# acg-team/ProGraphMSA

Hardware: AMD Instinct MI355X
Metric: DP cell-updates/sec (GCUPS) + wall-clock on 256 seqs × 1000 aa, WAG (higher is better)
Workload: dtype f32

## Files before the change

include/pgm_hip.h:

```cpp
#ifndef PGM_HIP_H_
#define PGM_HIP_H_

#include <stdint.h>
#include <stddef.h>

#ifdef __cplusplus
extern "C" {
#endif

#define PGM_OK 0
#define PGM_ERR_INVALID 1
#define PGM_ERR_DEVICE 2
#define PGM_ERR_BACKTRACK 3
#define PGM_ERR_NOMEM 4

#define PGM_GAP 0xFFFFFFFFu


typedef struct pgm_graph {
    uint32_t n;
    uint32_t dim;
    const double *sites;
    const int32_t *e_rowptr;
    const uint32_t *e_col;
// ... 63 lines not shown
                         float *ms_emission, float *ms_fill, float *ms_traceback);
int pgm_align_batch_stage_times(pgm_align_batch *b, int reset, float *ms_prep, float *ms_emission, float *ms_fill,
                                uint32_t *launches);
int pgm_align_batch_job_times(pgm_ctx *ctx, pgm_align_batch *b, uint64_t *ticks);
int pgm_align_batch_test_stall(pgm_align_batch *b, uint32_t job, uint32_t band, uint32_t spin_limit);
int pgm_test_cu_shares(uint32_t cus, double lean_cost, uint32_t nlean, double band_cost, uint32_t nbands, double rest_cost,
                       uint32_t nrest, uint32_t ncrit, double longest_chain, uint32_t *out4);
#define PGM_PLAN_HEAD 23
#define PGM_PLAN_DHEAD 9
#define PGM_PLAN_JOB 19
int pgm_test_batch_plan(uint32_t njobs, const pgm_graph *const *g1, const pgm_graph *const *g2, const pgm_model *const *model,
                        const pgm_scores *scores, uint32_t flags, const pgm_site_ref *res1, const pgm_site_ref *res2, uint32_t cus,
                        uint32_t *head, double *dhead, uint32_t *job_fields, uint32_t *items, uint32_t *bands, uint32_t *lean_list, int32_t *tblist);
int pgm_align_batch_read_matrices(pgm_ctx *ctx, pgm_align_batch *b, uint32_t job, float *M,
                                  float *X, float *Y, float *W, float *S);

int pgm_nw_pairs_batch(pgm_ctx *ctx, uint32_t dim, const int32_t *score, int32_t gap_open,
                       int32_t gap_extend, uint32_t nseq, const int8_t *syms,
                       const uint32_t *offs, uint32_t npairs, const uint32_t *pi,
                       const uint32_t *pj, int32_t *counts, uint32_t *gaps);
#define PGM_NW_REDUCED 1u
int pgm_nw_pairs_submit(pgm_ctx *ctx, uint32_t dim, const int32_t *score, int32_t gap_open,
                        int32_t gap_extend, uint32_t nseq, const int8_t *syms,
                        const uint32_t *offs, uint32_t npairs, const uint32_t *pi,
                        const uint32_t *pj, uint32_t flags, int32_t *counts, uint32_t *gaps, int *ticket);
int pgm_nw_pairs_wait(pgm_ctx *ctx, int ticket);
float pgm_nw_last_kernel_ms(pgm_ctx *ctx);
void *pgm_host_alloc(size_t bytes);
void pgm_host_free(void *p);

// ... 114 lines not shown
```

prographmsa_amd/__init__.py:

```python
import ctypes as C
import os

_HERE = os.path.dirname(os.path.abspath(__file__))
LIB_PATH = os.path.join(_HERE, "lib", "libpgm_hip.so")
PGMSA_PATH = os.path.join(_HERE, "bin", "pgmsa")

PGM_OK, PGM_ERR_INVALID, PGM_ERR_DEVICE, PGM_ERR_BACKTRACK, PGM_ERR_NOMEM = 0, 1, 2, 3, 4
PGM_GAP = 0xFFFFFFFF
PGM_BATCH_KEEP_MATRICES = 1
PGM_NW_REDUCED = 1
PGM_MERGE_RESIDENT = 1


class pgm_graph(C.Structure):
    _fields_ = [("n", C.c_uint32), ("dim", C.c_uint32), ("sites", C.POINTER(C.c_double)),
                ("e_rowptr", C.POINTER(C.c_int32)), ("e_col", C.POINTER(C.c_uint32)), ("e_val", C.POINTER(C.c_float)),
                ("r_rowptr", C.POINTER(C.c_int32)), ("r_col", C.POINTER(C.c_uint32)), ("r_units", C.POINTER(C.c_uint32))]


class pgm_model(C.Structure):
    _fields_ = [("M", C.POINTER(C.c_double)), ("pi", C.POINTER(C.c_double))]


class pgm_scores(C.Structure):
# ... 34 lines not shown
    _fields_ = [("index1", C.c_uint32), ("index2", C.c_uint32), ("dist1", C.c_double), ("dist2", C.c_double)]


class pgm_bionj_pair(C.Structure):
    _fields_ = [("index1", C.c_uint32), ("index2", C.c_uint32)]


class pgm_align_out(C.Structure):
    _fields_ = [("score", C.c_float), ("n_tr_indels", C.c_uint32), ("len", C.c_uint32), ("status", C.c_int32),
                ("map1", C.POINTER(C.c_uint32)), ("map2", C.POINTER(C.c_uint32))]


EXPORTS = [
    "pgm_device_count", "pgm_ctx_create", "pgm_ctx_destroy", "pgm_last_error", "pgm_ctx_device_info",
    "pgm_align_graphs_batch", "pgm_align_batch_create", "pgm_align_batch_create_ex", "pgm_align_batch_create_res", "pgm_align_graphs_batch_res", "pgm_align_batch_run", "pgm_align_batch_fetch",
    "pgm_align_batch_destroy", "pgm_align_batch_cells", "pgm_align_batch_test_stall", "pgm_test_cu_shares", "pgm_test_batch_plan", "pgm_align_batch_stage_times", "pgm_align_batch_job_times", "pgm_align_batch_time", "pgm_align_batch_read_matrices",
    "pgm_nw_pairs_batch", "pgm_nw_pairs_submit", "pgm_nw_pairs_wait", "pgm_nw_last_kernel_ms", "pgm_host_alloc", "pgm_host_free", "pgm_csprofile_load", "pgm_csprofile_create_batch", "pgm_csprofile_create_batch_res",
    "pgm_csprofile_last_kernel_ms", "pgm_mldist_batch", "pgm_prealigned_counts_batch", "pgm_kmer_cosine", "pgm_dist_last_kernel_ms",
    "pgm_kmer_cosine_multi", "pgm_prealigned_counts_multi", "pgm_prealigned_counts_resampled",
    "pgm_merge_profiles_batch", "pgm_merge_profiles_batch_ex", "pgm_resident_reset", "pgm_resident_onehot", "pgm_resident_import", "pgm_merge_last_kernel_ms",
    "pgm_gapmask_extend_batch", "pgm_gap_parsimony_batch", "pgm_parsimony_last_kernel_ms",
    "pgm_wls_load", "pgm_wls_pair_sums_batch", "pgm_wls_last_kernel_ms", "pgm_wls_last_launches",
    "pgm_bionj", "pgm_bionj_multi", "pgm_bionj_last_launches", "pgm_bionj_last_kernel_ms",
    "pgm_bionj_plan", "pgm_bionj_plan_multi",
    "pgm_msa_agreement", "pgm_agreement_last_kernel_ms",
    "pgm_transfer_min", "pgm_transfer_last_kernel_ms", "pgm_transfer_taxa",
]


def _load():
    if not os.path.exists(LIB_PATH):
# ... 13 lines not shown
        "pgm_align_batch_create_ex": (C.c_int, [vp, u32, PG, PG, PM, C.POINTER(pgm_scores), u32, C.POINTER(vp)]),
        "pgm_align_batch_create_res": (C.c_int, [vp, u32, PG, PG, PM, C.POINTER(pgm_scores), u32, C.POINTER(pgm_site_ref), C.POINTER(pgm_site_ref), C.POINTER(vp)]),
        "pgm_align_graphs_batch_res": (C.c_int, [vp, u32, PG, PG, PM, C.POINTER(pgm_scores), C.POINTER(pgm_site_ref), C.POINTER(pgm_site_ref), C.POINTER(pgm_align_out)]),
        "pgm_align_batch_run": (C.c_int, [vp, vp]),
        "pgm_align_batch_fetch": (C.c_int, [vp, vp, C.POINTER(pgm_align_out)]),
        "pgm_align_batch_destroy": (None, [vp, vp]),
        "pgm_align_batch_cells": (C.c_uint64, [vp]),
        "pgm_align_batch_test_stall": (C.c_int, [vp, u32, u32, u32]),
        "pgm_test_cu_shares": (C.c_int, [u32, C.c_double, u32, C.c_double, u32, C.c_double, u32, u32, C.c_double, C.POINTER(C.c_uint32)]),
        "pgm_test_batch_plan": (C.c_int, [u32, PG, PG, PM, C.POINTER(pgm_scores), u32, C.POINTER(pgm_site_ref), C.POINTER(pgm_site_ref), u32,
                                          C.POINTER(u32), C.POINTER(C.c_double)] + [C.POINTER(u32)] * 4 + [C.POINTER(i32)]),
        "pgm_align_batch_stage_times": (C.c_int, [vp, C.c_int] + [C.POINTER(C.c_float)] * 3 + [C.POINTER(u32)]),
        "pgm_align_batch_job_times": (C.c_int, [vp, vp, C.POINTER(C.c_uint64)]),
        "pgm_align_batch_time": (C.c_int, [vp, vp, C.c_int] + [C.POINTER(C.c_float)] * 4),
        "pgm_align_batch_read_matrices": (C.c_int, [vp, vp, u32] + [C.POINTER(C.c_float)] * 5),
        "pgm_nw_pairs_batch": (C.c_int, [vp, u32, C.POINTER(i32), i32, i32, u32, C.POINTER(C.c_int8), C.POINTER(u32), u32,
                                         C.POINTER(u32), C.POINTER(u32), C.POINTER(i32), C.POINTER(u32)]),
        "pgm_nw_pairs_submit": (C.c_int, [vp, u32, C.POINTER(i32), i32, i32, u32, C.POINTER(C.c_int8), C.POINTER(u32), u32,
                                          C.POINTER(u32), C.POINTER(u32), u32, C.POINTER(i32), C.POINTER(u32), C.POINTER(C.c_int)]),
        "pgm_nw_pairs_wait": (C.c_int, [vp, C.c_int]),
        "pgm_host_alloc": (vp, [C.c_size_t]),
        "pgm_host_free": (None, [vp]),
        "pgm_nw_last_kernel_ms": (C.c_float, [vp]),
        "pgm_csprofile_load": (C.c_int, [vp, u32, u32] + [C.POINTER(C.c_double)] * 3),
        "pgm_csprofile_create_batch": (C.c_int, [vp, u32, C.POINTER(C.c_int8), C.POINTER(u32)] + [C.POINTER(C.c_double)] * 4
                                       + [C.POINTER(C.c_uint64)]),
        "pgm_csprofile_create_batch_res": (C.c_int, [vp, u32, C.POINTER(C.c_int8), C.POINTER(u32)] + [C.POINTER(C.c_double)] * 3
                                           + [C.POINTER(C.POINTER(C.c_double))]),
        "pgm_csprofile_last_kernel_ms": (C.c_float, [vp]),
        "pgm_mldist_batch": (C.c_int, [vp, C.POINTER(pgm_mldist_model), u32, C.POINTER(i32), C.POINTER(u32)] + [C.POINTER(C.c_double)] * 3),
# ... 137 lines not shown
```

prographmsa_amd/csrc/pgm_align_kernels.h:

```cpp
#ifndef PGM_ALIGN_KERNELS_H_
#define PGM_ALIGN_KERNELS_H_

#include <hip/hip_runtime.h>
#include <math.h>
#include <type_traits>
#include "pgm_device.h"

#define PGM_NEG_INF (-INFINITY)

__device__ __forceinline__ float pgm_ls_log_add(float x, float add) {
    const float a = 2.44247459618085927548717403238913328776812604856113966238617812902399112761292613763080658235564f;
    const float b = -4.2040783745848554315883301529007786406310628696382695994938550046831869207082846248658671f;
    const float c = -0.72123729809042963774358701619456664388406302428056983119308906451199556380646306f;
    const uint32_t bits = __float_as_uint(x);
    const float e = (float)((int32_t)(bits >> 23) - 126);
    const float d = __uint_as_float(((bits << 9) >> 9) ^ 0x3f000000u);
    float t = __fdiv_rn(b, __fsub_rn(d, c));
    const float u = __fadd_rn(e, a);
    t = __fadd_rn(t, add);
    t = __fadd_rn(t, u);
    return t;
}

__device__ __forceinline__ float pgm_emission_finish(float num, float ay, float bx, float match_init) {
// ... 150 lines not shown
template <class T> __device__ __forceinline__ T pgm_gld(const T *p) { return *(const PGM_GLOBAL T *)(uintptr_t)p; }
#define PGM_EM_TB 4
template <int DP, int RB>
__global__ void __launch_bounds__(4 * PGM_ROWS) pgm_emission_skew_kernel(const PgmJob *__restrict__ jobs) {
    typedef float pgm_v2f __attribute__((ext_vector_type(2)));
    constexpr int NT = DP / 4;
    constexpr int COLS = 64 + PGM_EM_TB * PGM_BLOCK - PGM_HALO - 1;
    constexpr int STR = DP + 1;
    __shared__ pgm_v2f tp[(COLS + 1) * STR];
    __shared__ float bq[COLS];
    const PgmJob &J = jobs[blockIdx.z];
    const uint32_t tb0 = blockIdx.x * PGM_EM_TB;
    const uint32_t rsh = J.rshift, nvb = J.nb << rsh;
    if (tb0 >= J.nblk || 4u * RB * blockIdx.y >= nvb) return;
    if (J.tabhdr && pgm_gld(J.tabhdr) == 0) return;
    auto row_of = [&](uint32_t v, uint32_t lane_) { return ((((v >> rsh) << 6) + lane_) << rsh) | (v & ((1u << rsh) - 1u)); };
    auto sblock_of = [&](uint32_t v, uint32_t tb_) { return ((((size_t)(v >> rsh) * J.nblk + tb_) << rsh) | (v & ((1u << rsh) - 1u))); };
    const uint32_t t0 = tb0 * PGM_BLOCK;
    const int cbase = (int)t0 - 63;
    if ((DP == 20 || DP == 4) && RB == 1) {
        constexpr int TE = DP + 1;
        float *const tab = (float *)tp;
        static_assert(COLS * TE <= (COLS + 1) * STR * 2, "score table must fit the column staging area");
        static_assert(DP > 20 || TE <= 32, "row classes must fit As");
        __shared__ float As[32];
        const uint32_t fb0 = 4u * blockIdx.y + threadIdx.x / PGM_ROWS;
        const uint32_t fl = threadIdx.x % PGM_ROWS;
        const bool active = fb0 < nvb;
        int sym = DP;
        bool plain = true;
// ... 112 lines not shown
                }
            }
#pragma unroll
            for (int r = 0; r < RB; ++r) {
                out[r][i] = pgm_emission_finish(acc[r].x, ay[r], bq[ci], mi);
                out[r][i + 1] = pgm_emission_finish(acc[r].y, ay[r], bq[ci + 1], mi);
            }
        }
#pragma unroll
        for (int r = 0; r < RB; ++r) {
            if (b0 + (uint32_t)r < nvb) {
                PGM_GLOBAL pgm_v4f *dst = Sq + (sblock_of(b0 + (uint32_t)r, tb) * 64u + (uint32_t)l) * (PGM_BLOCK / 4);
#pragma unroll
                for (int q = 0; q < PGM_BLOCK / 4; ++q) dst[q] = pgm_v4f{out[r][4 * q], out[r][4 * q + 1], out[r][4 * q + 2], out[r][4 * q + 3]};
            }
        }
    }
}

__device__ __forceinline__ int pgm_wave_max8(uint32_t v) {
    int m = __builtin_amdgcn_ballot_w64(v >= 8u) != 0 ? 8 : 0;
    m += __builtin_amdgcn_ballot_w64(v >= (uint32_t)(m + 4)) != 0 ? 4 : 0;
    m += __builtin_amdgcn_ballot_w64(v >= (uint32_t)(m + 2)) != 0 ? 2 : 0;
    m += __builtin_amdgcn_ballot_w64(v >= (uint32_t)(m + 1)) != 0 ? 1 : 0;
    return m;
}

__device__ __forceinline__ __amdgpu_buffer_rsrc_t pgm_band_rsrc(float4 *base, uint32_t bytes) {
    const uint64_t p = (uint64_t)base;
    const uint32_t lo = __builtin_amdgcn_readfirstlane((uint32_t)p), hi = __builtin_amdgcn_readfirstlane((uint32_t)(p >> 32));
// ... 2249 lines not shown
```

prographmsa_amd/csrc/pgm_capi.hip:

```cpp
#include <hip/hip_runtime.h>

#include <algorithm>
#include <cmath>
#include <cstdio>
#include <thread>
#include <atomic>
#include <chrono>
#include <queue>
#include <cstdlib>
#include <cstring>
#include <numeric>
#include <mutex>
#include <string>
#include <unordered_set>
#include <vector>
#include <sys/mman.h>

#include "pgm_align_kernels.h"
#include "pgm_crit_kernels.h"
#include "pgm_nw_kernels.h"
#include "pgm_csprofile_kernels.h"
#include "pgm_dist_kernels.h"
#include "pgm_merge_kernels.h"
#include "pgm_parsimony_kernels.h"
// ... 14 lines not shown
            return fail(PGM_ERR_DEVICE, std::string(#x) + ": " + hipGetErrorString(e_));            \
    } while (0)

struct PgmNwState;
struct pgm_ctx {
    int device = 0;
    PgmNwState *nw = nullptr;
    int nw_per_cu = 0;
    struct ResChunk { uint8_t *p; size_t cap; };
    std::vector<ResChunk> res_chunks;
    size_t res_chunk = 0, res_off = 0;
    hipStream_t stream = nullptr;
    hipStream_t stream2 = nullptr;
    hipStream_t stream3 = nullptr;
    hipStream_t stream4 = nullptr;
    enum { C_IN, C_WORK, C_CELLS, C_OUT, C_S, C_HOST, C_HIN, C_SMALL, C_SLOTS };
    void *cache_ptr[C_SLOTS] = {};
    size_t cache_bytes[C_SLOTS] = {};
    hipDeviceProp_t prop;
    float nw_ms = 0, cs_ms = 0, ml_ms = 0, merge_ms = 0, pars_ms = 0, wls_ms = 0;
    uint32_t wls_n = 0, wls_launches = 0;
    float bionj_ms = 0;
    float agree_ms = 0;
    float transfer_ms = 0;
    uint32_t bionj_launches = 0;
    enum { SC_DEV = 36, SC_HOST = 4 };
    void *sc_dev[SC_DEV] = {};
    size_t sc_dev_bytes[SC_DEV] = {};
    void *sc_host[SC_HOST] = {};
    size_t sc_host_bytes[SC_HOST] = {};
    hipEvent_t sc_ev[2] = {nullptr, nullptr};
// ... 40 lines not shown

struct pgm_align_batch {
    uint32_t njobs = 0;
    uint64_t cells = 0;
    uint32_t maxdim = 0, maxnb = 0, maxn = 0, maxnblk = 0;
    std::vector<PgmJob> jobs;
    std::vector<uint32_t> order;
    BatchSchedule sched;
    uint8_t *d_in = nullptr;
    uint8_t *d_work = nullptr;
    uint8_t *d_cells = nullptr;
    uint8_t *d_out = nullptr;
    uint8_t *d_S = nullptr;
    uint8_t *d_small = nullptr;
    size_t in_bytes = 0, work_bytes = 0, cell_bytes = 0, out_bytes = 0, s_bytes = 0, small_bytes = 0;
    size_t cap[8] = {0, 0, 0, 0, 0, 0, 0, 0};
    uint8_t *h_out = nullptr;
    uint8_t *h_in = nullptr;
    int *h_flag = nullptr;
    int *d_sync = nullptr;
    size_t sync_ints = 0;
    uint32_t lq_off = 0;
    PgmJob *d_jobs = nullptr;
    uint32_t *d_order = nullptr;
    PgmItem *d_items = nullptr;
    uint32_t *d_lean = nullptr;
    PgmItem *d_bands = nullptr;
    int2 *d_tblist = nullptr;
    unsigned long long *d_times = nullptr;
    int *d_tabhdr = nullptr;
    hipEvent_t ev_fork = nullptr, ev_join = nullptr;
// ... 60 lines not shown
    (void)lib_pool().run(64, 16u, [](size_t) {});
    {
        void *p = nullptr;
        const size_t sb = (size_t)128 << 20;
        if (!getenv("PGM_NO_STAGING_RESERVE") && pinned_alloc(sb, &p) == hipSuccess) { c->cache_ptr[pgm_ctx::C_HIN] = p; c->cache_bytes[pgm_ctx::C_HIN] = sb; }
        else (void)hipGetLastError();
        const size_t rb = (size_t)8 << 20;
        if (!getenv("PGM_NO_STAGING_RESERVE") && hipHostMalloc(&p, rb, hipHostMallocDefault) == hipSuccess) { c->cache_ptr[pgm_ctx::C_HOST] = p; c->cache_bytes[pgm_ctx::C_HOST] = rb; }
        else (void)hipGetLastError();
        if (!getenv("PGM_NO_STAGING_RESERVE") && !getenv("PGM_NO_DEVICE_RESERVE")) {
            for (const BatchBuffer &e : kBatchBuffers) {
                void *d = nullptr;
                if (hipMalloc(&d, e.reserve_mb << 20) == hipSuccess) { c->cache_ptr[e.slot] = d; c->cache_bytes[e.slot] = e.reserve_mb << 20; }
                else { (void)hipGetLastError(); break; }
            }
        }
    }
    *out = c;
    return PGM_OK;
}

static void nw_state_free(PgmNwState *st);
void pgm_ctx_destroy(pgm_ctx *ctx) {
    if (!ctx) return;
    (void)hipSetDevice(ctx->device);
    nw_state_free(ctx->nw);
    for (auto &c : ctx->res_chunks) if (c.p) (void)hipFree(c.p);
    if (ctx->cs_lprofiles) (void)hipFree(ctx->cs_lprofiles);
    if (ctx->cs_centre) (void)hipFree(ctx->cs_centre);
    if (ctx->cs_priors) (void)hipFree(ctx->cs_priors);
// ... 90 lines not shown
    return {tier, threads, ((size_t)maxdim * maxdim + maxdim + threads * ((size_t)maxdim + 1)) * sizeof(float)};
}
static hipError_t launch_all(pgm_ctx *ctx, pgm_align_batch *b, bool timed) {
    hipStream_t s = ctx->stream;
    const BatchSchedule &S = b->sched;
    hipError_t e;
    for (uint32_t i = 0; i < b->njobs; ++i) ((PgmJob::Result *)(b->h_out + b->res_off[i]))->status = PGM_STATUS_PENDING;
    if (timed && (e = hipEventRecord(b->ev[0], s)) != hipSuccess) return e;
    const PrepTier T = prep_tier(b->maxdim);
    const dim3 pg(b->njobs, 2, (b->maxn + T.threads - 1) / T.threads);
    if (T.tier == 4) hipLaunchKernelGGL((pgm_prep_kernel<4, 256>), pg, dim3(256), T.lds, s, b->d_jobs, b->d_sync, (uint32_t)b->sync_ints);
    else if (T.tier == 20) hipLaunchKernelGGL((pgm_prep_kernel<20, 256>), pg, dim3(256), T.lds, s, b->d_jobs, b->d_sync, (uint32_t)b->sync_ints);
    else hipLaunchKernelGGL((pgm_prep_kernel<64, 64>), pg, dim3(64), T.lds, s, b->d_jobs, b->d_sync, (uint32_t)b->sync_ints);
    if ((e = hipGetLastError()) != hipSuccess) return e;
    if (timed && (e = hipEventRecord(b->ev[1], s)) != hipSuccess) return e;
    const dim3 eg((b->maxnblk + PGM_EM_TB - 1) / PGM_EM_TB, (b->maxnb + 3) / 4, b->njobs);
    if (T.tier == 4) hipLaunchKernelGGL((pgm_emission_skew_kernel<4, 1>), eg, dim3(4 * PGM_ROWS), 0, s, b->d_jobs);
    else if (T.tier == 20) hipLaunchKernelGGL((pgm_emission_skew_kernel<20, 1>), eg, dim3(4 * PGM_ROWS), 0, s, b->d_jobs);
    else hipLaunchKernelGGL((pgm_emission_skew_kernel<64, 1>), eg, dim3(4 * PGM_ROWS), 0, s, b->d_jobs);
    if ((e = hipGetLastError()) != hipSuccess) return e;
    if (timed && (e = hipEventRecord(b->ev[2], s)) != hipSuccess) return e;
    const uint32_t spin_limit = b->test_spin_limit ? b->test_spin_limit : PGM_SPIN_LIMIT, stall_job = b->test_stall_job, stall_band = b->test_stall_band;
    const bool fork = S.nlean != 0;
    const bool bandk = S.nbands != 0;
    const bool tbk = (S.nitems != 0 || bandk) && (S.ntb + S.ntb_c + S.ntb_b) != 0;
    const bool critk = S.ncrit != 0;
    if ((fork || bandk || critk) && (e = hipEventRecord(b->ev_fork, s)) != hipSuccess) return e;
    if (critk && (e = hipStreamWaitEvent(ctx->stream4, b->ev_fork, 0)) != hipSuccess) return e;
    if (fork && (e = hipStreamWaitEvent(ctx->stream2, b->ev_fork, 0)) != hipSuccess) return e;
    if (bandk && (e = hipStreamWaitEvent(ctx->stream3, b->ev_fork, 0)) != hipSuccess) return e;
// ... 89 lines not shown
        if (e3 == hipSuccess) b->h_flag = (int *)(b->h_out + (b->out_bytes + 15) / 16 * 16);
        if (e3 == hipSuccess) e3 = hipHostGetDevicePointer((void **)&A->h_out_dev, b->h_out, 0);
        A->host_err = e3;
    }
    A->ms_host = now_ms() - ta0 - A->ms_dev;
}

struct CreateGuard {
    pgm_ctx *ctx;
    pgm_align_batch *b;
    std::thread alloc;
    ~CreateGuard() { if (alloc.joinable()) alloc.join(); if (b) pgm_align_batch_destroy(ctx, b); }
    pgm_align_batch *release() { pgm_align_batch *r = b; b = nullptr; return r; }
};

static void bind_job_pointers(pgm_align_batch *b, const std::vector<JobOff> &off, const pgm_site_ref *res1, const pgm_site_ref *res2, uint8_t *h_out_dev) {
    for (uint32_t i = 0; i < b->njobs; ++i) {
        PgmJob &J = b->jobs[i];
        const JobOff &o = off[i];
        uint8_t *in = b->d_in, *w = b->d_work, *ob = b->d_out;
        J.sites1 = site_ref_of(res1, i) ? res1[i].dev_sites : (const double *)(in + o.s1.sites);
        J.sites2 = site_ref_of(res2, i) ? res2[i].dev_sites : (const double *)(in + o.s2.sites);
        J.smap1 = o.s1.has_smap ? (const uint32_t *)(in + o.s1.smap) : nullptr;
        J.smap2 = o.s2.has_smap ? (const uint32_t *)(in + o.s2.smap) : nullptr;
        J.M = (const double *)(in + o.M); J.pi = (const double *)(in + o.pi);
        J.ni1 = (const PgmNode2 *)(in + o.s1.ni); J.ni2 = (const PgmNode2 *)(in + o.s2.ni);
        J.xp1 = (const int32_t *)(in + o.s1.xp); J.xp2 = (const int32_t *)(in + o.s2.xp);
        J.xc1 = (const uint32_t *)(in + o.s1.xc); J.xc2 = (const uint32_t *)(in + o.s2.xc);
        J.xv1 = (const float *)(in + o.s1.xv); J.xv2 = (const float *)(in + o.s2.xv);
        J.fp1 = (const int32_t *)(in + o.s1.fp); J.fe1 = (const uint2 *)(in + o.s1.fe);
        J.ov2 = (const uint2 *)(in + o.s2.ov);
        J.pp1 = (const int32_t *)(in + o.s1.pp); J.pp2 = (const int32_t *)(in + o.s2.pp);
        J.pc1 = (const uint32_t *)(in + o.s1.pc); J.pc2 = (const uint32_t *)(in + o.s2.pc);
// ... 129 lines not shown
            int st;
            while ((st = A.state.load(std::memory_order_acquire)) == 0) std::this_thread::yield();
            if (st == 1) {
                (void)hipSetDevice(ctx->device);
                const hipError_t eu = hipMemcpyAsync(b->d_in + in_base[c0], b->h_in + in_base[c0], in_base[c1] - in_base[c0], hipMemcpyHostToDevice, ctx->stream);
                if (eu != hipSuccess) upload_err.store((int)eu);
            }
        }
    });
    if (bad.load() >= 0) return fail(PGM_ERR_INVALID, "invalid graph in job " + std::to_string(bad.load()));
    const double tc2 = now_ms();
    G.alloc.join();
    const double tc3 = now_ms();
    if (A.err != hipSuccess) return fail(A.err == hipErrorOutOfMemory ? PGM_ERR_NOMEM : PGM_ERR_DEVICE, std::string("hipMalloc: ") + hipGetErrorString(A.err));
    if (A.host_err != hipSuccess) return fail(PGM_ERR_DEVICE, std::string("hipHostMalloc: ") + hipGetErrorString(A.host_err));
    bind_job_pointers(b, Z.off, res1, res2, A.h_out_dev);
    b->order = size_order(b->jobs);
    b->sched = plan_schedule(b->jobs, b->order, cus);
    const BatchSchedule &S = b->sched;
    if (cprof && njobs)
        fprintf(stderr, "    work lists: longest chain of sweeps %.0f us, goal %.0f us; lean %zu jobs %.0f us-worker on %u CUs; bands %zu, %.0f us-worker on %u CUs (simulated end %.0f us); items %zu, %.0f us-worker on %u CUs (simulated end %.0f us), of the longest chains %zu on %u CUs (%.0f us)\n",
                S.rsweep, S.t_goal, (size_t)S.nlean, S.lean_cost, S.nlean_workers, S.total_b, S.band_cost, S.nband_workers, S.band_end, S.total, S.other_cost, S.capacity, S.fill_end, S.total_c, S.ncrit_workers, S.crit_end);
    const double tc4 = now_ms();
    if (S.nitems > std::max<size_t>(1, sm.total_bands)) return fail(PGM_ERR_DEVICE, "work list longer than the number of bands");
    if ((e = (hipError_t)upload_err.load()) != hipSuccess ||
        (e = hipMemcpyAsync(b->d_tblist, S.tblist.data(), 8 * S.tblist.size(), hipMemcpyHostToDevice, ctx->stream)) != hipSuccess ||
        (e = hipMemcpyAsync(b->d_jobs, b->jobs.data(), sizeof(PgmJob) * njobs, hipMemcpyHostToDevice, ctx->stream)) != hipSuccess ||
        (e = hipMemcpyAsync(b->d_order, b->order.data(), 4 * (size_t)njobs, hipMemcpyHostToDevice, ctx->stream)) != hipSuccess ||
        (e = hipMemcpyAsync(b->d_items, S.items.data(), sizeof(PgmItem) * S.items.size(), hipMemcpyHostToDevice, ctx->stream)) != hipSuccess ||
        (e = hipMemcpyAsync(b->d_lean, S.lean_list.data(), 4 * S.lean_list.size(), hipMemcpyHostToDevice, ctx->stream)) != hipSuccess ||
// ... 119 lines not shown
}

void pgm_align_batch_destroy(pgm_ctx *ctx, pgm_align_batch *b) {
    if (!b) return;
    if (ctx) { (void)hipSetDevice(ctx->device); (void)hipStreamSynchronize(ctx->stream); }
    if (ctx && ctx->stream2) (void)hipStreamSynchronize(ctx->stream2);
    if (ctx && ctx->stream3) (void)hipStreamSynchronize(ctx->stream3);
    if (ctx && ctx->stream4) (void)hipStreamSynchronize(ctx->stream4);
    for (int k = 0; k < 5; ++k)
        if (b->ev[k]) (void)hipEventDestroy(b->ev[k]);
    if (b->ev_fork) (void)hipEventDestroy(b->ev_fork);
    if (b->ev_join) (void)hipEventDestroy(b->ev_join);
    if (b->ev_join_b) (void)hipEventDestroy(b->ev_join_b);
    if (b->ev_join_c) (void)hipEventDestroy(b->ev_join_c);
    for (const BatchBuffer &e : kBatchBuffers) cache_give(ctx, e.slot, b->*e.ptr, b->cap[e.slot]);
    cache_give(ctx, pgm_ctx::C_HOST, b->h_out, b->cap[pgm_ctx::C_HOST]);
    cache_give(ctx, pgm_ctx::C_HIN, b->h_in, b->cap[pgm_ctx::C_HIN]);
    delete b;
}

uint64_t pgm_align_batch_cells(const pgm_align_batch *b) { return b ? b->cells : 0; }

int pgm_align_batch_stage_times(pgm_align_batch *b, int reset, float *ms_prep, float *ms_emission, float *ms_fill, uint32_t *launches) {
    if (!b) return fail(PGM_ERR_INVALID, "null batch");
    const double n = b->acc_n ? (double)b->acc_n : 1.0;
    if (ms_prep) *ms_prep = (float)(b->acc_ms[0] / n);
    if (ms_emission) *ms_emission = (float)(b->acc_ms[1] / n);
    if (ms_fill) *ms_fill = (float)(b->acc_ms[2] / n);
    if (launches) *launches = b->acc_n;
    if (reset) { b->acc_ms[0] = b->acc_ms[1] = b->acc_ms[2] = 0; b->acc_n = 0; }
// ... 21 lines not shown
    if (rc != PGM_OK) return rc;
    const auto t1 = std::chrono::steady_clock::now();
    {
        static std::mutex device_turn[64];
        std::lock_guard<std::mutex> turn(device_turn[(unsigned)ctx->device % 64u]);
        rc = pgm_align_batch_run(ctx, b);
        if (rc == PGM_OK) rc = pgm_align_batch_fetch(ctx, b, out);
    }
    const auto t2 = std::chrono::steady_clock::now();
    pgm_align_batch_destroy(ctx, b);
    if (prof)
        fprintf(stderr, "  pgm_align_graphs_batch: %u jobs, create (flatten, allocate, upload, work list) %.2f ms, run + fetch %.2f ms, destroy %.2f ms\n", njobs,
                std::chrono::duration<double, std::milli>(t1 - t0).count(), std::chrono::duration<double, std::milli>(t2 - t1).count(),
                std::chrono::duration<double, std::milli>(std::chrono::steady_clock::now() - t2).count());
    return rc;
}

int pgm_align_batch_read_matrices(pgm_ctx *ctx, pgm_align_batch *b, uint32_t job, float *M, float *X, float *Y, float *W, float *S) {
    if (!ctx || !b || job >= b->njobs) return fail(PGM_ERR_INVALID, "bad argument");
    HIPCHK(hipSetDevice(ctx->device));
    HIPCHK(hipStreamSynchronize(ctx->stream));
    const PgmJob &J = b->jobs[job];
    const size_t N = (size_t)J.n1 * J.n2;
    if ((M || X || Y || W) && !J.keep_cells)
        return fail(PGM_ERR_INVALID, "the DP matrices of a chain-only job are only kept for a batch created with PGM_BATCH_KEEP_MATRICES");
    if (S && J.tabhdr) {
        int bad = 1;
        HIPCHK(hipMemcpy(&bad, J.tabhdr, sizeof(int), hipMemcpyDeviceToHost));
        if (bad == 0) return fail(PGM_ERR_INVALID, "the score matrix of a job of two sequence graphs is only stored for a batch created with PGM_BATCH_KEEP_MATRICES");
    }
// ... 47 lines not shown
```

prographmsa_amd/csrc/pgm_device.h:

```cpp
#ifndef PGM_DEVICE_H_
#define PGM_DEVICE_H_

#include <stdint.h>
#include "../../include/pgm_hip.h"

#define PGM_MAX_DIM 64
#define PGM_HALO 0
#define PGM_ROWS 64
#define PGM_VL 16
#define PGM_BLOCK 8
#define PGM_NRING 128
#define PGM_KF 4
#define PGM_KF8 8
#define PGM_DCAP 28
#define PGM_PF 4
#define PGM_REMOTE_MAX 128
#define PGM_WAVES 8
#define PGM_WIDE_WAVES 4
#define PGM_POOL 163584
#define PGM_CPARTS 3
#define PGM_AUX_RES 0
#define PGM_AUX_SBLK 3072
#define PGM_AUX_EL 9216
#define PGM_AUX_CNT 13312
// ... 12 lines not shown
    float cc, c2, c3;
    uint32_t flags;
    uint32_t fd[PGM_KF8];
    float fc[PGM_KF8];
};

#define PGM_TB_PK 8
struct PgmTbNode {
    uint32_t cnt;
    uint32_t c[PGM_TB_PK];
    float v[PGM_TB_PK];
    uint32_t u[PGM_TB_PK];
    uint32_t pad[7];
};

struct PgmJob {
    uint32_t n1, n2;
    uint32_t dim, dp;
    uint32_t nb;
    uint32_t ncol;
    uint32_t tsteps;
    uint32_t maxn;
    uint32_t has_extras;
    uint32_t has_far;
    uint32_t mode2;
    uint32_t far_slack;
    uint32_t aux_off;
    uint32_t hD, hDX;
    uint32_t slot_bytes;
    uint32_t nslots;
// ... 19 lines not shown
    const int32_t *pp1, *pp2;
    const uint32_t *pc1, *pc2;
    const float *pv1, *pv2;
    const uint32_t *pu1, *pu2;

    PgmTbNode *tb1, *tb2;
    float *g1f;
    float *a1;
    float *t2;
    float *b2;

    float *S;
    uint32_t nblk;
    const uint8_t *cls1, *cls2;
    int *tabhdr;

    uint32_t *codes;
    float4 *endcell;
    uint32_t keep_cells;

    uint16_t *ltab;
    int *lready;
    uint32_t lrows, lcols;

    unsigned long long *times;

    float4 *cells;
    int *prog;

    uint32_t *map1, *map2;
// ... 35 lines not shown
```

Baseline: 81.08.

## Deduplicate identical emission profiles via hashed classes and expand from a compact table

```diff
diff --git a/include/pgm_hip.h b/include/pgm_hip.h
--- a/include/pgm_hip.h
+++ b/include/pgm_hip.h
@@ -101,6 +101,7 @@
                         uint32_t *head, double *dhead, uint32_t *job_fields, uint32_t *items, uint32_t *bands, uint32_t *lean_list, int32_t *tblist);
 int pgm_align_batch_read_matrices(pgm_ctx *ctx, pgm_align_batch *b, uint32_t job, float *M,
                                   float *X, float *Y, float *W, float *S);
+int pgm_align_batch_emission_classes(pgm_ctx *ctx, pgm_align_batch *b, uint32_t *out);
 
 int pgm_nw_pairs_batch(pgm_ctx *ctx, uint32_t dim, const int32_t *score, int32_t gap_open,
                        int32_t gap_extend, uint32_t nseq, const int8_t *syms,
diff --git a/prographmsa_amd/__init__.py b/prographmsa_amd/__init__.py
--- a/prographmsa_amd/__init__.py
+++ b/prographmsa_amd/__init__.py
@@ -72,7 +72,7 @@
 EXPORTS = [
     "pgm_device_count", "pgm_ctx_create", "pgm_ctx_destroy", "pgm_last_error", "pgm_ctx_device_info",
     "pgm_align_graphs_batch", "pgm_align_batch_create", "pgm_align_batch_create_ex", "pgm_align_batch_create_res", "pgm_align_graphs_batch_res", "pgm_align_batch_run", "pgm_align_batch_fetch",
-    "pgm_align_batch_destroy", "pgm_align_batch_cells", "pgm_align_batch_test_stall", "pgm_test_cu_shares", "pgm_test_batch_plan", "pgm_align_batch_stage_times", "pgm_align_batch_job_times", "pgm_align_batch_time", "pgm_align_batch_read_matrices",
+    "pgm_align_batch_destroy", "pgm_align_batch_cells", "pgm_align_batch_test_stall", "pgm_test_cu_shares", "pgm_test_batch_plan", "pgm_align_batch_stage_times", "pgm_align_batch_job_times", "pgm_align_batch_time", "pgm_align_batch_read_matrices", "pgm_align_batch_emission_classes",
     "pgm_nw_pairs_batch", "pgm_nw_pairs_submit", "pgm_nw_pairs_wait", "pgm_nw_last_kernel_ms", "pgm_host_alloc", "pgm_host_free", "pgm_csprofile_load", "pgm_csprofile_create_batch", "pgm_csprofile_create_batch_res",
     "pgm_csprofile_last_kernel_ms", "pgm_mldist_batch", "pgm_prealigned_counts_batch", "pgm_kmer_cosine", "pgm_dist_last_kernel_ms",
     "pgm_kmer_cosine_multi", "pgm_prealigned_counts_multi", "pgm_prealigned_counts_resampled",
@@ -116,6 +116,7 @@
         "pgm_align_batch_job_times": (C.c_int, [vp, vp, C.POINTER(C.c_uint64)]),
         "pgm_align_batch_time": (C.c_int, [vp, vp, C.c_int] + [C.POINTER(C.c_float)] * 4),
         "pgm_align_batch_read_matrices": (C.c_int, [vp, vp, u32] + [C.POINTER(C.c_float)] * 5),
+        "pgm_align_batch_emission_classes": (C.c_int, [vp, vp, C.POINTER(u32)]),
         "pgm_nw_pairs_batch": (C.c_int, [vp, u32, C.POINTER(i32), i32, i32, u32, C.POINTER(C.c_int8), C.POINTER(u32), u32,
                                          C.POINTER(u32), C.POINTER(u32), C.POINTER(i32), C.POINTER(u32)]),
         "pgm_nw_pairs_submit": (C.c_int, [vp, u32, C.POINTER(i32), i32, i32, u32, C.POINTER(C.c_int8), C.POINTER(u32), u32,
diff --git a/prographmsa_amd/csrc/pgm_align_kernels.h b/prographmsa_amd/csrc/pgm_align_kernels.h
--- a/prographmsa_amd/csrc/pgm_align_kernels.h
+++ b/prographmsa_amd/csrc/pgm_align_kernels.h
@@ -188,6 +188,7 @@
     const uint32_t rsh = J.rshift, nvb = J.nb << rsh;
     if (tb0 >= J.nblk || 4u * RB * blockIdx.y >= nvb) return;
     if (J.tabhdr && pgm_gld(J.tabhdr) == 0) return;
+    if (pgm_gld(&J.emrec->use) != 0u) return;
     auto row_of = [&](uint32_t v, uint32_t lane_) { return ((((v >> rsh) << 6) + lane_) << rsh) | (v & ((1u << rsh) - 1u)); };
     auto sblock_of = [&](uint32_t v, uint32_t tb_) { return ((((size_t)(v >> rsh) * J.nblk + tb_) << rsh) | (v & ((1u << rsh) - 1u))); };
     const uint32_t t0 = tb0 * PGM_BLOCK;
@@ -330,6 +331,163 @@
 #pragma unroll
                 for (int q = 0; q < PGM_BLOCK / 4; ++q) dst[q] = pgm_v4f{out[r][4 * q], out[r][4 * q + 1], out[r][4 * q + 2], out[r][4 * q + 3]};
             }
+        }
+    }
+}
+
+template <int DP>
+__global__ void __launch_bounds__(1024) pgm_emission_classify_kernel(const PgmJob *__restrict__ jobs) {
+    __shared__ uint32_t slot[PGM_EMC_SLOTS];
+    __shared__ uint16_t nslot[PGM_EMC_MAXN];
+    __shared__ uint32_t count;
+    const PgmJob &J = jobs[blockIdx.x];
+    const bool first = blockIdx.y == 0;
+    uint32_t *const cnt_out = first ? &J.emrec->c1 : &J.emrec->c2;
+    if (J.lean || J.n1 > PGM_EMC_MAXN || J.n2 > PGM_EMC_MAXN) {
+        if (threadIdx.x == 0) *cnt_out = 0u;
+        return;
+    }
+    const uint32_t n = first ? J.n1 - 1u : J.n2;
+    const float *const prof = first ? J.g1f : J.t2, *const den = first ? J.a1 : J.b2;
+    uint16_t *const cls = first ? J.emc1 : J.emc2, *const rep = first ? J.emr1 : J.emr2;
+    for (uint32_t i = threadIdx.x; i < PGM_EMC_SLOTS; i += 1024u) slot[i] = 0u;
+    if (threadIdx.x == 0) count = 0u;
+    __syncthreads();
+    for (uint32_t v = threadIdx.x; v < n; v += 1024u) {
+        uint32_t key[DP + 1];
+        const uint4 *src = (const uint4 *)(prof + (size_t)DP * v);
+#pragma unroll
+        for (int q = 0; q < DP / 4; ++q) {
+            const uint4 w = src[q];
+            key[4 * q] = w.x; key[4 * q + 1] = w.y; key[4 * q + 2] = w.z; key[4 * q + 3] = w.w;
+        }
+        key[DP] = __float_as_uint(pgm_gld(den + v));
+        uint32_t h = 2166136261u;
+#pragma unroll
+        for (int k = 0; k <= DP; ++k) h = (h ^ key[k]) * 16777619u;
+        uint32_t s = (h ^ (h >> 15)) & (PGM_EMC_SLOTS - 1u);
+        for (;;) {
+            const uint32_t old = atomicCAS(&slot[s], 0u, v + 1u);
+            if (old == 0u) break;
+            const uint4 *oth = (const uint4 *)(prof + (size_t)DP * (old - 1u));
+            bool same = key[DP] == __float_as_uint(pgm_gld(den + (old - 1u)));
+#pragma unroll
+            for (int q = 0; q < DP / 4; ++q) {
+                const uint4 w = oth[q];
+                same = same && key[4 * q] == w.x && key[4 * q + 1] == w.y && key[4 * q + 2] == w.z && key[4 * q + 3] == w.w;
+            }
+            if (same) break;
+            s = (s + 1u) & (PGM_EMC_SLOTS - 1u);
+        }
+        nslot[v] = (uint16_t)s;
+    }
+    __syncthreads();
+    for (uint32_t i = threadIdx.x; i < PGM_EMC_SLOTS; i += 1024u) {
+        const uint32_t o = slot[i];
+        if (o != 0u) {
+            const uint32_t id = atomicAdd(&count, 1u);
+            rep[id] = (uint16_t)(o - 1u);
+            slot[i] = id;
+        }
+    }
+    __syncthreads();
+    for (uint32_t v = threadIdx.x; v < n; v += 1024u) cls[v] = (uint16_t)slot[nslot[v]];
+    if (threadIdx.x == 0) *cnt_out = count;
+}
+
+template <int DP>
+__global__ void __launch_bounds__(256) pgm_emission_table_kernel(const PgmJob *__restrict__ jobs) {
+    __shared__ float gl[64 * DP];
+    __shared__ float al[64];
+    const PgmJob &J = jobs[blockIdx.y];
+    const uint32_t c1 = pgm_gld(&J.emrec->c1), c2 = pgm_gld(&J.emrec->c2);
+    const bool use = pgm_emc_eligible(J.n1, J.n2, c1, c2);
+    if (blockIdx.x == 0 && threadIdx.x == 0) J.emrec->use = use ? 1u : 0u;
+    if (!use) return;
+    const uint32_t W = c2 + 1u, ntc = (W + 63u) / 64u, ntiles = ntc * ((c1 + 63u) / 64u);
+    const uint32_t lane = threadIdx.x & 63u, wave = threadIdx.x >> 6;
+    const float mi = J.sc.match_init;
+    PGM_GLOBAL float *const tab = (PGM_GLOBAL float *)(uintptr_t)J.cells;
+    for (uint32_t tile = blockIdx.x; tile < ntiles; tile += gridDim.x) {
+        const uint32_t r0 = (tile / ntc) * 64u, c = (tile % ntc) * 64u + lane;
+        const uint32_t nr = min(64u, c1 - r0);
+        __syncthreads();
+        for (uint32_t i = threadIdx.x; i < nr * (DP / 4); i += 256u) {
+            const uint32_t node = pgm_gld(J.emr1 + r0 + i / (DP / 4));
+            ((float4 *)gl)[i] = ((const float4 *)(J.g1f + (size_t)DP * node))[i % (DP / 4)];
+        }
+        if (threadIdx.x < nr) al[threadIdx.x] = pgm_gld(J.a1 + pgm_gld(J.emr1 + r0 + threadIdx.x));
+        float t[DP], b = 0.f;
+#pragma unroll
+        for (int k = 0; k < DP; ++k) t[k] = 0.f;
+        if (c < c2) {
+            const uint32_t node = pgm_gld(J.emr2 + c);
+            const float4 *src = (const float4 *)(J.t2 + (size_t)DP * node);
+#pragma unroll
+            for (int q = 0; q < DP / 4; ++q) {
+                const float4 w = src[q];
+                t[4 * q] = w.x; t[4 * q + 1] = w.y; t[4 * q + 2] = w.z; t[4 * q + 3] = w.w;
+            }
+            b = pgm_gld(J.b2 + node);
+        }
+        __syncthreads();
+        if (c < W) {
+            for (uint32_t r = wave; r < nr; r += 4u) {
+                const float *g = gl + r * DP;
+                float acc = 0.0f;
+#pragma unroll
+                for (int k = 0; k < DP; ++k) acc = __fadd_rn(acc, __fmul_rn(g[k], t[k]));
+                tab[(size_t)(r0 + r) * W + c] = pgm_emission_finish(acc, al[r], b, mi);
+            }
+        }
+    }
+}
+
+__global__ void __launch_bounds__(256) pgm_emission_expand_kernel(const PgmJob *__restrict__ jobs) {
+    extern __shared__ __attribute__((aligned(16))) unsigned char emx_lds[];
+    __shared__ uint32_t rcls[64];
+    const PgmJob &J = jobs[blockIdx.y];
+    if (pgm_gld(&J.emrec->use) == 0u) return;
+    const uint32_t rsh = J.rshift, nvb = J.nb << rsh;
+    const uint32_t c2 = pgm_gld(&J.emrec->c2), W = c2 + 1u, G = pgm_emc_rows(c2, J.n2);
+    const uint32_t gsh = 31u - (uint32_t)__builtin_clz(G), per_band = 64u >> gsh, nunits = nvb * per_band;
+    if (blockIdx.x >= nunits) return;
+    auto row_of = [&](uint32_t v_, uint32_t lane_) { return ((((v_ >> rsh) << 6) + lane_) << rsh) | (v_ & ((1u << rsh) - 1u)); };
+    auto sblock_of = [&](uint32_t v_, uint32_t tb_) { return ((((size_t)(v_ >> rsh) * J.nblk + tb_) << rsh) | (v_ & ((1u << rsh) - 1u))); };
+    float *const rows = (float *)emx_lds;
+    uint16_t *const cl2 = (uint16_t *)(emx_lds + (size_t)G * W * sizeof(float));
+    const uint32_t ncol = J.ncol, n1 = J.n1, nblk = J.nblk, total = nblk << gsh;
+    for (uint32_t i = threadIdx.x; i <= ncol; i += 256u) cl2[i] = pgm_gld(J.emc2 + i);
+    const PGM_GLOBAL float *const tab = (const PGM_GLOBAL float *)(uintptr_t)J.cells;
+    PGM_GLOBAL pgm_v4f *const Sq = (PGM_GLOBAL pgm_v4f *)(uintptr_t)J.S;
+    for (uint32_t unit = blockIdx.x; unit < nunits; unit += gridDim.x) {
+        const uint32_t v = unit >> (6u - gsh), l0 = (unit & (per_band - 1u)) << gsh;
+        __syncthreads();
+        if (threadIdx.x < G) {
+            const uint32_t y = row_of(v, l0 + threadIdx.x);
+            rcls[threadIdx.x] = pgm_gld(J.emc1 + ((y + 1 < n1) ? y : 0u));
+        }
+        __syncthreads();
+#pragma unroll 4
+        for (uint32_t i = threadIdx.x; i < G * W; i += 256u) {
+            const uint32_t g = i / W;
+            rows[i] = tab[(size_t)rcls[g] * W + (i - g * W)];
+        }
+        __syncthreads();
+#pragma unroll 2
+        for (uint32_t idx = threadIdx.x; idx < total; idx += 256u) {
+            const uint32_t g = idx & (G - 1u), tb = idx >> gsh, l = l0 + g;
+            const float *row = rows + g * W;
+            const int x0 = (int)(tb * PGM_BLOCK) - (int)l;
+            float out[PGM_BLOCK];
+#pragma unroll
+            for (int i = 0; i < PGM_BLOCK; ++i) {
+                const int x = x0 + i;
+                out[i] = row[(x >= 0 && x <= (int)ncol) ? (uint32_t)cl2[x] : c2];
+            }
+            PGM_GLOBAL pgm_v4f *dst = Sq + (sblock_of(v, tb) * 64u + l) * (PGM_BLOCK / 4);
+#pragma unroll
+            for (int q = 0; q < PGM_BLOCK / 4; ++q) dst[q] = pgm_v4f{out[4 * q], out[4 * q + 1], out[4 * q + 2], out[4 * q + 3]};
         }
     }
 }
diff --git a/prographmsa_amd/csrc/pgm_capi.hip b/prographmsa_amd/csrc/pgm_capi.hip
--- a/prographmsa_amd/csrc/pgm_capi.hip
+++ b/prographmsa_amd/csrc/pgm_capi.hip
@@ -52,7 +52,7 @@
     hipStream_t stream2 = nullptr;
     hipStream_t stream3 = nullptr;
     hipStream_t stream4 = nullptr;
-    enum { C_IN, C_WORK, C_CELLS, C_OUT, C_S, C_HOST, C_HIN, C_SMALL, C_SLOTS };
+    enum { C_IN, C_WORK, C_CELLS, C_OUT, C_S, C_HOST, C_HIN, C_SMALL, C_EMC, C_SLOTS };
     void *cache_ptr[C_SLOTS] = {};
     size_t cache_bytes[C_SLOTS] = {};
     hipDeviceProp_t prop;
@@ -123,7 +123,9 @@
     uint8_t *d_S = nullptr;
     uint8_t *d_small = nullptr;
     size_t in_bytes = 0, work_bytes = 0, cell_bytes = 0, out_bytes = 0, s_bytes = 0, small_bytes = 0;
-    size_t cap[8] = {0, 0, 0, 0, 0, 0, 0, 0};
+    uint8_t *d_emc = nullptr;
+    size_t emc_bytes = 0;
+    size_t cap[pgm_ctx::C_SLOTS] = {};
     uint8_t *h_out = nullptr;
     uint8_t *h_in = nullptr;
     int *h_flag = nullptr;
@@ -214,6 +216,9 @@
                 if (hipMalloc(&d, e.reserve_mb << 20) == hipSuccess) { c->cache_ptr[e.slot] = d; c->cache_bytes[e.slot] = e.reserve_mb << 20; }
                 else { (void)hipGetLastError(); break; }
             }
+            void *d = nullptr;
+            if (hipMalloc(&d, (size_t)4 << 20) == hipSuccess) { c->cache_ptr[pgm_ctx::C_EMC] = d; c->cache_bytes[pgm_ctx::C_EMC] = (size_t)4 << 20; }
+            else (void)hipGetLastError();
         }
     }
     *out = c;
@@ -334,6 +339,19 @@
     else hipLaunchKernelGGL((pgm_prep_kernel<64, 64>), pg, dim3(64), T.lds, s, b->d_jobs, b->d_sync, (uint32_t)b->sync_ints);
     if ((e = hipGetLastError()) != hipSuccess) return e;
     if (timed && (e = hipEventRecord(b->ev[1], s)) != hipSuccess) return e;
+    const dim3 cg(b->njobs, 2), tg(PGM_EMC_TABLE_WG, b->njobs), xg(PGM_EMC_EXPAND_WG, b->njobs);
+    if (T.tier == 4) {
+        hipLaunchKernelGGL((pgm_emission_classify_kernel<4>), cg, dim3(1024), 0, s, b->d_jobs);
+        hipLaunchKernelGGL((pgm_emission_table_kernel<4>), tg, dim3(256), 0, s, b->d_jobs);
+    } else if (T.tier == 20) {
+        hipLaunchKernelGGL((pgm_emission_classify_kernel<20>), cg, dim3(1024), 0, s, b->d_jobs);
+        hipLaunchKernelGGL((pgm_emission_table_kernel<20>), tg, dim3(256), 0, s, b->d_jobs);
+    } else {
+        hipLaunchKernelGGL((pgm_emission_classify_kernel<64>), cg, dim3(1024), 0, s, b->d_jobs);
+        hipLaunchKernelGGL((pgm_emission_table_kernel<64>), tg, dim3(256), 0, s, b->d_jobs);
+    }
+    hipLaunchKernelGGL(pgm_emission_expand_kernel, xg, dim3(256), PGM_EMC_LDS, s, b->d_jobs);
+    if ((e = hipGetLastError()) != hipSuccess) return e;
     const dim3 eg((b->maxnblk + PGM_EM_TB - 1) / PGM_EM_TB, (b->maxnb + 3) / 4, b->njobs);
     if (T.tier == 4) hipLaunchKernelGGL((pgm_emission_skew_kernel<4, 1>), eg, dim3(4 * PGM_ROWS), 0, s, b->d_jobs);
     else if (T.tier == 20) hipLaunchKernelGGL((pgm_emission_skew_kernel<20, 1>), eg, dim3(4 * PGM_ROWS), 0, s, b->d_jobs);
@@ -453,9 +471,23 @@
     pgm_align_batch *release() { pgm_align_batch *r = b; b = nullptr; return r; }
 };
 
+static size_t emc_job_bytes(const PgmJob &J) { return J.lean ? 0 : (4 * ((size_t)J.n1 + J.n2) + 15) / 16 * 16; }
+static size_t emc_layout(const std::vector<PgmJob> &jobs) {
+    size_t off = (sizeof(PgmEmClasses) * jobs.size() + 15) / 16 * 16;
+    for (const PgmJob &J : jobs) off += emc_job_bytes(J);
+    return off;
+}
+
 static void bind_job_pointers(pgm_align_batch *b, const std::vector<JobOff> &off, const pgm_site_ref *res1, const pgm_site_ref *res2, uint8_t *h_out_dev) {
+    size_t emc = (sizeof(PgmEmClasses) * b->jobs.size() + 15) / 16 * 16;
     for (uint32_t i = 0; i < b->njobs; ++i) {
         PgmJob &J = b->jobs[i];
+        J.emrec = (PgmEmClasses *)b->d_emc + i;
+        if (!J.lean) {
+            uint16_t *p = (uint16_t *)(b->d_emc + emc);
+            J.emc1 = p; J.emc2 = p + J.n1; J.emr1 = p + J.n1 + J.n2; J.emr2 = p + 2 * (size_t)J.n1 + J.n2;
+            emc += emc_job_bytes(J);
+        }
         const JobOff &o = off[i];
         uint8_t *in = b->d_in, *w = b->d_work, *ob = b->d_out;
         J.sites1 = site_ref_of(res1, i) ? res1[i].dev_sites : (const double *)(in + o.s1.sites);
@@ -615,6 +647,9 @@
     const double tc3 = now_ms();
     if (A.err != hipSuccess) return fail(A.err == hipErrorOutOfMemory ? PGM_ERR_NOMEM : PGM_ERR_DEVICE, std::string("hipMalloc: ") + hipGetErrorString(A.err));
     if (A.host_err != hipSuccess) return fail(PGM_ERR_DEVICE, std::string("hipHostMalloc: ") + hipGetErrorString(A.host_err));
+    b->emc_bytes = std::max<size_t>(emc_layout(b->jobs), 16);
+    if ((e = cache_take(ctx, pgm_ctx::C_EMC, b->emc_bytes, (void **)&b->d_emc, &b->cap[pgm_ctx::C_EMC])) != hipSuccess)
+        return fail(e == hipErrorOutOfMemory ? PGM_ERR_NOMEM : PGM_ERR_DEVICE, std::string("hipMalloc: ") + hipGetErrorString(e));
     bind_job_pointers(b, Z.off, res1, res2, A.h_out_dev);
     b->order = size_order(b->jobs);
     b->sched = plan_schedule(b->jobs, b->order, cus);
@@ -764,6 +799,7 @@
     if (b->ev_join_b) (void)hipEventDestroy(b->ev_join_b);
     if (b->ev_join_c) (void)hipEventDestroy(b->ev_join_c);
     for (const BatchBuffer &e : kBatchBuffers) cache_give(ctx, e.slot, b->*e.ptr, b->cap[e.slot]);
+    cache_give(ctx, pgm_ctx::C_EMC, b->d_emc, b->cap[pgm_ctx::C_EMC]);
     cache_give(ctx, pgm_ctx::C_HOST, b->h_out, b->cap[pgm_ctx::C_HOST]);
     cache_give(ctx, pgm_ctx::C_HIN, b->h_in, b->cap[pgm_ctx::C_HIN]);
     delete b;
@@ -815,6 +851,16 @@
                 std::chrono::duration<double, std::milli>(t1 - t0).count(), std::chrono::duration<double, std::milli>(t2 - t1).count(),
                 std::chrono::duration<double, std::milli>(std::chrono::steady_clock::now() - t2).count());
     return rc;
+}
+
+int pgm_align_batch_emission_classes(pgm_ctx *ctx, pgm_align_batch *b, uint32_t *out) {
+    if (!ctx || !b || (b->njobs && !out)) return fail(PGM_ERR_INVALID, "null argument");
+    HIPCHK(hipSetDevice(ctx->device));
+    HIPCHK(hipStreamSynchronize(ctx->stream));
+    std::vector<PgmEmClasses> rec(b->njobs);
+    if (b->njobs) HIPCHK(hipMemcpy(rec.data(), b->d_emc, sizeof(PgmEmClasses) * b->njobs, hipMemcpyDeviceToHost));
+    for (uint32_t i = 0; i < b->njobs; ++i) { out[3 * i] = rec[i].use; out[3 * i + 1] = rec[i].c1; out[3 * i + 2] = rec[i].c2; }
+    return PGM_OK;
 }
 
 int pgm_align_batch_read_matrices(pgm_ctx *ctx, pgm_align_batch *b, uint32_t job, float *M, float *X, float *Y, float *W, float *S) {
diff --git a/prographmsa_amd/csrc/pgm_device.h b/prographmsa_amd/csrc/pgm_device.h
--- a/prographmsa_amd/csrc/pgm_device.h
+++ b/prographmsa_amd/csrc/pgm_device.h
@@ -50,6 +50,21 @@
     uint32_t pad[7];
 };
 
+struct PgmEmClasses { uint32_t use, c1, c2, pad; };
+#define PGM_EMC_SLOTS 8192u
+#define PGM_EMC_MAXN 4096u
+#define PGM_EMC_LDS 32768u
+#define PGM_EMC_EXPAND_WG 64u
+#define PGM_EMC_TABLE_WG 128u
+__host__ __device__ inline uint32_t pgm_emc_rows(uint32_t c2, uint32_t n2) {
+    for (uint32_t g = 64u; g >= 8u; g >>= 1)
+        if ((uint64_t)g * (c2 + 1u) * 4u + 2u * (uint64_t)n2 <= (uint64_t)PGM_EMC_LDS) return g;
+    return 0u;
+}
+__host__ __device__ inline bool pgm_emc_eligible(uint32_t n1, uint32_t n2, uint32_t c1, uint32_t c2) {
+    return c1 != 0u && c2 != 0u && 2ull * c1 * c2 <= (uint64_t)(n1 - 1u) * (n2 - 1u) && pgm_emc_rows(c2, n2) != 0u;
+}
+
 struct PgmJob {
     uint32_t n1, n2;
     uint32_t dim, dp;
@@ -99,6 +114,8 @@
     uint32_t nblk;
     const uint8_t *cls1, *cls2;
     int *tabhdr;
+    uint16_t *emc1, *emc2, *emr1, *emr2;
+    PgmEmClasses *emrec;
 
     uint32_t *codes;
     float4 *endcell;
```

Result: slower. 79.91 (-1.4%).
